# blyssprivacy/sdk

Measured on AMD Instinct MI355X. Metric: PIR queries/sec (full answer path) on 2^20 items x 256 B, higher is better.
Workload: dtype u64; 1 GPU; spiral-rs process_query, c2 = {"db_item_size": 256, "instances": 1, "n": 2, "nu_1": 9, "nu_2": 11, "p": 256, "q2_bits": 20, "t_conv": 4, "t_exp_left": 8, "t_exp_right": 56, "t_gsw": 8}, encoded DB 64.0 GiB (56.0 GiB resident per GPU), unsharded, one query per step

## Files before the change

### sdk_amd/csrc/fold.hip

```cpp
#include <type_traits>

#include "device_common.hpp"
#include "wave_ntt.hpp"
#include "bodies.hpp"

namespace spiral {

__device__ __forceinline__ bool fold_zero_shortcut(const u64* ct0, const u64* ct1, u64* out, int tau) {
  int nz0 = 0, nz1 = 0;
#pragma unroll
  for (int k = 0; k < 16; k++) {
    nz0 |= ct0[tau + 256 * k] != 0;
    nz1 |= ct1[tau + 256 * k] != 0;
  }
  const int any0 = __syncthreads_or(nz0), any1 = __syncthreads_or(nz1);
  if (any0 && any1) return false;
  const u64* src = any0 ? ct0 : ct1;
#pragma unroll
  for (int k = 0; k < 16; k++) out[tau + 256 * k] = src[tau + 256 * k];
  return true;
}

__global__ __launch_bounds__(256, 2) void k_fold_fused(DevTables T, FoldDesc d) {
  __shared__ u32 lds0[LDS_WORDS];
  __shared__ u32 lds1[LDS_WORDS];
  const int tau = threadIdx.x;
  const int i = (int)blockIdx.x, plane = blockIdx.y;
  const int two_t = 2 * d.t, four_t = 4 * d.t;
  const int t_live = d.t_live > 0 && d.t_live < d.t ? d.t_live : d.t;
  const u64* ct0 = d.X + ((size_t)plane * d.cur + i) * 2 * N;
  const u64* ct1 = ct0 + (size_t)d.half * 2 * N;
  const u64 mask = (1ULL << d.bits) - 1ULL;
  u32* la = lds0;
  u32* lb = lds1;
  u64* out = d.Y + ((size_t)plane * d.half + i) * 2 * N;
  if (d.zero_shortcuts && fold_zero_shortcut(ct0, ct1, out, tau)) return;
#pragma unroll 1
// ... 406 lines not shown
      } else {
#pragma unroll
        for (int kk = 0; kk < 16; kk++) mine_out[64 * kk + lt] = rr[kk];
      }
      __syncthreads();
      {
        const u32* theirs = exch + (irow * 2 + (1 - imod)) * (N / 2);
        u64* orow = out + (size_t)irow * N + (size_t)khalf * 1024;
        const u32 q0 = T.c.mod[0].q, q1 = T.c.mod[1].q;
        auto compose = [&](auto mod1_wave) {
          constexpr bool M1 = decltype(mod1_wave)::value;
#pragma unroll
          for (int kk = 0; kk < 16; kk++) {
            const u32 other = theirs[64 * kk + lt];
            const u32 own = rr[M1 ? kk : 16 + kk];
            const u32 x = M1 ? other : own, y = M1 ? own : other;
            const u32 xm = x >= q1 ? x - q1 : x;
            const u32 dd = y >= xm ? y - xm : y + q1 - xm;
            const u32 qt = __umulhi(dd, T.c.q0_inv_q1_sh);
            u32 e = dd * T.c.q0_inv_q1 - qt * q1;
            e = e >= q1 ? e - q1 : e;
            const u64 val = (u64)x + (u64)q0 * (u64)e + cpre[kk];
            const u64 res = val >= T.c.Q ? val - T.c.Q : val;
            orow[64 * kk + lt] = res;
          }
        };
        if (wv < 2) compose(std::true_type{});
        else compose(std::false_type{});
      }
    }
  }
}

__global__ __launch_bounds__(256, 2) void k_expand_wave(DevTables T, ExpandWaveDesc d, GroupOff g) {
  extern __shared__ __attribute__((aligned(16))) u32 smem_fw[];
  u32* wbuf = smem_fw;
  u32* ltw = smem_fw + 4 * WBUF_WORDS;
  u64* raw0 = reinterpret_cast<u64*>(ltw + 2 * N);
  const int tau = threadIdx.x, lane = tau & 63;
  const int wv = __builtin_amdgcn_readfirstlane(tau >> 6);
  const int b = (int)blockIdx.x, c = (int)blockIdx.y, qi = (int)blockIdx.z;
  const ModConst m = T.c.mod[c];
  const u32* fw = T.tw + (size_t)c * 4 * N;
  const u64* src = group_rebase(d.raw, g.raw[qi]) + (size_t)d.pos[b] * 2 * N;
  const u32* A_w = group_rebase(d.A_w, g.pp[qi]);
  u32* vout = group_rebase(d.v, g.v[qi]);
  u32* mybuf = wbuf + wv * WBUF_WORDS;
  wtw_stage(ltw, wave_fwd_image(T.tw, c), tau);
#pragma unroll
  for (int k = 0; k < 8; k++) raw0[tau + 256 * k] = src[tau + 256 * k];
  __syncthreads();
  const u64 mask = (1ULL << d.bits) - 1ULL;
  u64 acc0[32], acc1[32];
#pragma unroll
  for (int k = 0; k < 32; k++) acc0[k] = acc1[k] = 0;
#pragma unroll 1
  for (int dg = wv; dg <= d.t; dg += 4) {
    int ln = lane;
    const u32* fwi = fw;
    asm volatile("" : "+v"(ln));
    asm volatile("" : "+s"(fwi));
    WaveScalarTw stw;
    wntt_scalar_tw(stw, fwi);
    u32 v[32];
    if (dg < d.t) {
      const int sh = dg * d.bits;
// ... 54 lines not shown
      w.y = add_mod(wv == 0 ? r0[4 * g4 + 1] : r1[4 * g4 + 1], a.y, m.q);
      w.z = add_mod(wv == 0 ? r0[4 * g4 + 2] : r1[4 * g4 + 2], a.z, m.q);
      w.w = add_mod(wv == 0 ? r0[4 * g4 + 3] : r1[4 * g4 + 3], a.w, m.q);
      reinterpret_cast<uint4*>(o)[g4] = w;
    }
  }
}
void launch_expand_wave(const DevTables& T, const ExpandWaveDesc& d, const GroupOff& g, int B, hipStream_t s) {
  if (d.cnt <= 0 || B <= 0) return;
  const size_t lds = (size_t)(4 * WBUF_WORDS + 2 * N) * 4 + (size_t)N * 8;
  hipLaunchKernelGGL(k_expand_wave, dim3(d.cnt, 2, B), dim3(256), lds, s, T, d, g);
  launched(PATH_EXPAND_FUSED | PATH_EXPAND_WAVE, "k_expand_wave");
}

__global__ __launch_bounds__(256) void k_mats_to_wave(MatsToWaveDesc d) { mats_to_wave_body(d, blockIdx.x); }
void launch_mats_to_wave(u32* dst, const u32* src, size_t n_words, hipStream_t s, int half_polys) {
  if (n_words == 0) return;
  const MatsToWaveDesc d{dst, src, n_words, half_polys};
  hipLaunchKernelGGL(k_mats_to_wave, dim3((unsigned)((n_words + 255) / 256)), dim3(256), 0, s, d);
  launched(0, "k_mats_to_wave");
}

__global__ __launch_bounds__(256) void k_mats_to_wave_group(MatsToWaveDesc d, GroupOff g) {
  const int qi = blockIdx.y;
  d.dst = group_rebase(d.dst, g.raw[qi]);
  d.src = group_rebase(d.src, g.v[qi]);
  mats_to_wave_body(d, blockIdx.x);
}
void launch_mats_to_wave_group(u32* dst, const u32* src, size_t n_words, int half_polys, const GroupOff& g, int B, hipStream_t s) {
  if (n_words == 0 || B <= 0) return;
  const MatsToWaveDesc d{dst, src, n_words, half_polys};
  hipLaunchKernelGGL(k_mats_to_wave_group, dim3((unsigned)((n_words + 255) / 256), B), dim3(256), 0, s, d, g);
  launched(PATH_EXPAND_GROUP, "k_mats_to_wave_group");
}

void launch_fold_fused(const DevTables& T, const FoldDesc& d, hipStream_t s) {
  if (d.half <= 0 || d.planes <= 0) return;
  const int variant = (int)tunable("fold_variant", FOLD_VARIANT_DEFAULT);
  const dim3 grid(d.half, d.planes), block(256);
  if (variant == 5 && d.mats_w && d.bits <= 28) {
    const int es = d.bits <= 8 ? 1 : d.bits <= 16 ? 2 : 4;
    const int t_live = d.t_live > 0 && d.t_live < d.t ? d.t_live : d.t;
    const size_t lds = FOLD_WAVE_FIXED_LDS + (size_t)2 * t_live * (N * es + 256);
    if (lds <= 80 * 1024) {
      if (es == 1)
        hipLaunchKernelGGL(k_fold_wave<1>, grid, block, lds, s, T, d, d.mats_w);
      else if (es == 2)
        hipLaunchKernelGGL(k_fold_wave<2>, grid, block, lds, s, T, d, d.mats_w);
      else
        hipLaunchKernelGGL(k_fold_wave<4>, grid, block, lds, s, T, d, d.mats_w);
      launched(PATH_FOLD_FUSED | PATH_FOLD_WAVE, "k_fold_wave");
      return;
    }
  }
  if (variant != 0 && (d.t % 2) == 0)
    hipLaunchKernelGGL(k_fold_fused2, grid, block, 0, s, T, d);
  else
    hipLaunchKernelGGL(k_fold_fused, grid, block, 0, s, T, d);
  launched(PATH_FOLD_FUSED, "k_fold_fused");
}

}
```

### sdk_amd/csrc/kernels.hpp

```cpp
#pragma once
#include <hip/hip_runtime.h>

#include <vector>

#include "params.hpp"

namespace spiral {

constexpr int N = (int)POLY_LEN;

struct DevTables {
  const u32* tw;
  DevConsts c;
};
__host__ __device__ inline const u32* inv_tables(const u32* tw, int c) { return tw + (size_t)8 * N + (size_t)c * 2 * N; }
__host__ __device__ inline const u32* wave_fwd_image(const u32* tw, int c) { return tw + (size_t)12 * N + (size_t)c * 2 * N; }
__host__ __device__ inline int wtw_phys(int idx) {
  if (idx >= 1024) {
    const int L = (idx - 1024) >> 4, r = (idx - 1024) & 15;
    return 1024 + 16 * L + 4 * (((r >> 2) + (L >> 2)) & 3) + (r & 3);
  }
  if (idx >= 512) {
    const int L = (idx - 512) >> 3, r = (idx - 512) & 7;
    return 512 + 8 * L + 4 * (((r >> 2) + (L >> 3)) & 1) + (r & 3);
// ... 128 lines not shown
                               hipStream_t s);
void launch_reorient_group(u64* out, const u32* v, int first, int step, int dim0, const GroupOff& g, int B, hipStream_t s);
void launch_copy_polys_group(u32* dst, const int* dst_idx, int dst_row_stride, const u32* src, const int* src_idx, int src_row_stride,
                             int R, int batch, const GroupOff& g, int B, hipStream_t s);
void launch_folding_neg_group(const DevTables& T, u32* mats, const u32* gadget_ntt, int nu2, int two_t, const GroupOff& g, int B,
                              hipStream_t s);
void launch_mats_to_wave_group(u32* dst, const u32* src, size_t n_words, int half_polys, const GroupOff& g, int B, hipStream_t s);
struct ExpandWaveDesc {
  const u64* raw;
  const int* pos;
  const int* out_idx;
  const u32* A_w;
  const u32* const_w;
  u32* v;
  int cnt, t, bits;
};
void launch_expand_wave(const DevTables& T, const ExpandWaveDesc& d, const GroupOff& g, int B, hipStream_t s);
constexpr long EXPAND_WAVE_MIN_DIGITS_DEFAULT = 16;
constexpr long EXPAND_GROUP_ROUND_MIN_DEFAULT = 4096;

struct FoldDesc {
  const u64* X;
  u64* Y;
  const u32* mats;
  int cur, half, planes;
  int t, bits;
  int t_live;
  int zero_shortcuts;
  const u32* mats_w;
};
void launch_mats_to_wave(u32* dst, const u32* src, size_t n_words, hipStream_t s, int half_polys = 0);
constexpr long FOLD_VARIANT_DEFAULT = 5;
void launch_fold_fused(const DevTables& T, const FoldDesc& d, hipStream_t s);

void launch_add_poly_into(const DevTables& T, u32* dst, const int* idx, const u32* src, int batch, hipStream_t s);
void launch_scalar_mul(const DevTables& T, u32* base, long dst_off, long src_off, const u32* scalar, int n_polys,
                       hipStream_t s);
void launch_add_polys_idx(const DevTables& T, u32* dst, const int* di, const u32* a, const int* ai, const u32* b,
                          const int* bi, int count, hipStream_t s);
void launch_interleave_query(u64* qv, const u32* row0_ntt, const u64* wire, int dim0, hipStream_t s);
void launch_copy_polys(u32* dst, const int* dst_idx, int dst_row_stride, const u32* src, const int* src_idx,
                       int src_row_stride, int R, int batch, hipStream_t s);
void launch_folding_neg(const DevTables& T, u32* mats, const u32* gadget_ntt, int nu2, int two_t, hipStream_t s);
void launch_add(const DevTables& T, u32* out, const u32* a, const u32* b, int n_polys, hipStream_t s);
void launch_invert_raw(const DevTables& T, u64* out, const u64* a, long n_words, hipStream_t s);
void launch_automorph(const DevTables& T, u64* out, const u64* a, int n_polys, int t, hipStream_t s);
void launch_gadget_raw(u64* out, const u64* inp, int rows_in, int cols, int rows_out, int rdim, int bits,
                       hipStream_t s);
void launch_u64_to_u32(u32* out, const u64* in, long n, hipStream_t s);
void launch_u32_to_u64(u64* out, const u32* in, long n, hipStream_t s);

void launch_cu_probe(u32* out, int blocks, hipStream_t s);

struct EncodeDesc {
  const u64* packed;
  unsigned long long* out;
  int instances, n;
  u64 Q, q1, q2;
  int q1_bits, q2_bits;
};
void launch_encode(const EncodeDesc& d, hipStream_t s);

void launch_reorient(u64* out, const u32* v, int first, int step, int dim0, hipStream_t s);

struct CopyPolysDesc {
  u32* dst;
// ... 154 lines not shown
```

### sdk_amd/csrc/pipeline.hpp

```cpp
#pragma once
#include <vector>

#include "server.hpp"

namespace spiral {

struct Workspace {
  const Params* P;
  DeviceState* D;
  int device = -1;
  hipStream_t stream = nullptr;
  hipStream_t stream2 = nullptr;
  std::vector<hipEvent_t> ev_plane;
  hipEvent_t ev_fold = nullptr;
  hipEvent_t ev_round0 = nullptr, ev_right = nullptr;
  bool right_pending = false;
  bool long_sweep_follows = false;
  hipEvent_t ev_sw[2] = {nullptr, nullptr};
  bool have_sweep_span = false;
  bool pipelined = false;
  hipEvent_t ev[5] = {nullptr, nullptr, nullptr, nullptr, nullptr};
  DevBuf<u64> q_raw;
  DevBuf<u32> v;
  DevBuf<u64> exp_raw;
// ... 30 lines not shown
  ~Workspace();
  Workspace(const Workspace&) = delete;
  Workspace& operator=(const Workspace&) = delete;
  void ensure_expand();
  void ensure_sweep();
  void ensure_finish();
  size_t plane_group() const;
};

void run_coefficient_expansion(Workspace& W, const sp_pp& pp, size_t g_rounds, const DeviceState::PrunedPlan* plan = nullptr,
                               int tree = 0, size_t r_begin = 0);
void join_right(Workspace& W);
void run_regev_to_gsw(Workspace& W, const sp_pp& pp, const u32* v_src, const int* src_ct, const int* src_poly);
void run_folding_neg(Workspace& W);
void run_mats_to_wave(Workspace& W, size_t levels, bool c_only = false);
void run_fold_operands(Workspace& W);
void run_begin_direct(Workspace& W, const uint8_t* query);
void run_begin_group(Workspace* const* Ws, const sp_pp* const* pps, const uint8_t* const* queries, const size_t* query_lens, int B);
void run_begin(Workspace& W, const sp_pp& pp, const uint8_t* query, size_t query_len, int j0 = 0, int nj = 0,
               const DeviceState::PrunedPlan* plan = nullptr);
void run_sweep_sparse(Workspace& W, const sp_db& db, const int* col_ptr, const int* col_rows, const int* col_slots);
void run_sweep_sparse_group(Workspace* const* Ws, int B, const sp_db& db, const int* col_ptr, const int* col_rows, const int* col_slots,
                            hipStream_t s);
std::unique_ptr<DeviceState::PrunedPlan> build_pruned_plan_rows(const Params& P, const std::vector<char>& rows);
void run_sweep(Workspace& W, const sp_db& db);
void run_sweep_pipelined(Workspace& W, const sp_db& db);
bool sweep_is_pipelined(const Params& p, const sp_db& db);
void launch_plane_sweep(Workspace& W, const sp_db& db, size_t plane);
bool fused_fold_supported(const Params& p);
struct FoldOpts {
  long fused_min_pairs;
  bool delta_tail;
  bool inputs_below_q;
};
u64* run_fold(Workspace& W, const FoldOpts& o, u64* X, u64* Y, int np, int num_cts, int top, int d_begin = 0, int d_end = -1);
void run_fold_local(Workspace& W, const u32* reduced_chunk, int G);
void run_fold_local_plane(Workspace& W, const u32* reduced_plane_chunk, int G, int plane);
void run_fold_local_join(Workspace& W);
void run_finish_gathered(Workspace& W, const sp_pp& pp, const u64* gathered, int G);
void run_fold_all(Workspace& W, bool premod);
void run_pack(Workspace& W, const sp_pp& pp);
void run_finish(Workspace& W, const sp_pp& pp, bool premod);
size_t encode_response(const Params& p, const u64* packed, uint8_t* out);
void run_encode_device(Workspace& W);

}
```

### sdk_amd/csrc/server.cpp

```cpp
#include "server.hpp"

#include <algorithm>
#include <atomic>
#include <cstdlib>
#include <cstring>
#include <functional>

#include "pipeline.hpp"

namespace spiral {

void hip_check(hipError_t e, const char* what, const char* file, int line) {
  if (e != hipSuccess) {
    (void)hipGetLastError();
    throw HipError(std::string(what) + " failed at " + file + ":" + std::to_string(line) + ": " + hipGetErrorString(e));
  }
}

static std::mutex g_tun_mu;
static std::vector<std::pair<std::string, long>> g_tun;
static std::atomic<unsigned> g_tun_epoch{1};
static std::atomic<long> g_fresh_allocs{0};
void tunables_new_call() { g_tun_epoch.fetch_add(1, std::memory_order_relaxed); }
void set_tunable(const char* name, long v) {
// ... 1113 lines not shown
void join_right(Workspace& W) {
  if (W.right_pending) HIP_CHECK(hipStreamWaitEvent(W.stream, W.ev_right, 0));
}

void run_sweep(Workspace& W, const sp_db& db) {
  const Params& p = *W.P;
  W.ensure_sweep();
  SweepDesc d{db.words.p, W.qv.p, W.sweep_out.p, (int)p.planes(), db.np_local, (int)p.dim0(), db.j0, db.nj, db.packed, W.out_G};
  d.nt_store = (int)tunable("sweep_nt_store", 1);
  launch_sweep(W.D->T, d, W.stream);
}

void run_sweep_sparse(Workspace& W, const sp_db& db, const int* col_ptr, const int* col_rows, const int* col_slots) {
  const Params& p = *W.P;
  W.ensure_sweep();
  launch_sweep_sparse(W.D->T, col_ptr, col_rows, col_slots, db.polys.p, (int)p.planes(), W.v.p, 0,
                      p.db_dim_2 > 0 ? 2 : 1, W.sweep_out.p, (int)p.num_per(), W.stream);
}

void run_sweep_sparse_group(Workspace* const* Ws, int B, const sp_db& db, const int* col_ptr, const int* col_rows, const int* col_slots,
                            hipStream_t s) {
  const Params& p = *Ws[0]->P;
  SparseGroup g{};
  for (int b = 0; b < B; b++) {
    Ws[b]->ensure_sweep();
    g.v[b] = Ws[b]->v.p;
    g.out[b] = Ws[b]->sweep_out.p;
  }
  launch_sweep_sparse_batch(Ws[0]->D->T, col_ptr, col_rows, col_slots, db.polys.p, (int)p.planes(), g, B, 0, p.db_dim_2 > 0 ? 2 : 1,
                            (int)p.num_per(), s);
}

static FoldOpts query_fold_opts(const Workspace& W, bool below_q) {
  return FoldOpts{std::min(W.fused_min_pairs, tunable("fused_min_pairs_cap", 1L << 62)), true, below_q};
}

static void fold_planes(Workspace& W, size_t pg0, int np, bool premod) {
  const Params& p = *W.P;
  DeviceState& D = *W.D;
  hipStream_t s = W.stream;
  if (p.num_per() % 4 == 0 && !tunable("from_sweep1", 0)) {
    launch_from_sweep4(D.T, W.sweep_out.p + pg0 * 4 * POLY_LEN * p.num_per(), (int)p.num_per(), np, premod ? 1 : 0,
                       W.foldX.p, s);
  } else {
    InvDesc inv{};
    inv.src = W.sweep_out.p + pg0 * 4 * POLY_LEN * p.num_per();
    inv.sweep_np = (int)p.num_per();
    inv.dst = W.foldX.p;
    inv.n_polys = np * (int)p.num_per() * 2;
    inv.premod = premod ? 1 : 0;
    launch_ntt_inv(D.T, inv, s);
  }
  u64* res = run_fold(W, query_fold_opts(W, true), W.foldX.p, W.foldY.p, np, (int)p.num_per(), -1);
  HIP_CHECK(hipMemcpyAsync(W.final_cts.p + pg0 * 2 * POLY_LEN, res, (size_t)np * 2 * POLY_LEN * sizeof(u64), hipMemcpyDeviceToDevice, s));
}

static int tail_defer_levels(const Params& p, long stop) {
  if (stop <= 0 || !fused_fold_supported(p) || p.planes() < 2) return 0;
  int lv = 0;
  size_t cur = p.num_per();
  while (cur > (size_t)stop && cur / 2 >= 1 && (cur & 1) == 0) { cur >>= 1; lv++; }
  return cur == (size_t)stop && lv > 0 && stop >= 2 ? lv : 0;
}
static void fold_plane_head(Workspace& W, size_t pl, int levels) {
  const Params& p = *W.P;
  launch_from_sweep4(W.D->T, W.sweep_out.p + pl * 4 * POLY_LEN * p.num_per(), (int)p.num_per(), 1, 0, W.foldX.p, W.stream);
  u64* res = run_fold(W, query_fold_opts(W, true), W.foldX.p, W.foldY.p, 1, (int)p.num_per(), -1, 0, levels);
  const size_t cts = p.num_per() >> levels;
  HIP_CHECK(hipMemcpyAsync(W.fold_tail.p + pl * cts * 2 * POLY_LEN, res, cts * 2 * POLY_LEN * sizeof(u64), hipMemcpyDeviceToDevice, W.stream));
}
static void fold_tails(Workspace& W, int levels) {
  const Params& p = *W.P;
  const size_t cts = p.num_per() >> levels;
  u64* other = W.fold_tail.p + p.planes() * cts * 2 * POLY_LEN;
  u64* res = run_fold(W, query_fold_opts(W, true), W.fold_tail.p, other, (int)p.planes(), (int)p.num_per(), -1, levels, -1);
  HIP_CHECK(hipMemcpyAsync(W.final_cts.p, res, p.planes() * 2 * POLY_LEN * sizeof(u64), hipMemcpyDeviceToDevice, W.stream));
}

bool sweep_is_pipelined(const Params& p, const sp_db& db) {
  const bool enabled = tunable("pipeline", 1) != 0;
  return enabled && db.packed && db.num_shards == 1 && db.col_G == 1 && p.planes() > 1 && p.num_per() >= 1024;
}

void launch_plane_sweep(Workspace& W, const sp_db& db, size_t pl) {
  const Params& p = *W.P;
  const size_t np_ = (size_t)db.np_local;
  const size_t plane_db_words = db_bytes(1, db.np_local, db.nj, db.packed) / 8;
  SweepDesc d{db.words.p + pl * plane_db_words, W.qv.p, W.sweep_out.p + pl * 4 * POLY_LEN * np_, 1, db.np_local,
              (int)p.dim0(), db.j0, db.nj, db.packed, W.out_G};
  d.nt_store = (int)tunable("sweep_nt_store", 1);
  const int wgs = (int)tunable("pipe_wgs", 4);
  if (db.packed && wgs > 0)
    launch_sweep_persist(W.D->T, d, wgs, W.stream);
  else
    launch_sweep(W.D->T, d, W.stream);
}

void run_sweep_pipelined(Workspace& W, const sp_db& db) {
  const Params& p = *W.P;
  W.ensure_sweep();
  W.ensure_finish();
  const size_t planes = p.planes();
  HIP_CHECK(hipEventRecord(W.ev_sw[0], W.stream));
  const int defer_levels = tail_defer_levels(p, tunable("pipe_tail_defer", 256));
  if (defer_levels > 0) {
    W.fold_tail.ensure(2 * planes * (p.num_per() >> defer_levels) * 2 * POLY_LEN);
    note_path(PATH_FOLD_TAIL_BATCHED);
  }
  for (size_t pl = 0; pl < planes; pl++) {
    launch_plane_sweep(W, db, pl);
    HIP_CHECK(hipEventRecord(W.ev_plane[pl], W.stream));
    HIP_CHECK(hipStreamWaitEvent(W.stream2, W.ev_plane[pl], 0));
    if (defer_levels > 0) {
      on_stream(W, W.stream2, [&] {
        fold_plane_head(W, pl, defer_levels);
        if (pl + 1 == planes) fold_tails(W, defer_levels);
      });
      continue;
    }
    on_stream(W, W.stream2, [&] { fold_planes(W, pl, 1, false); });
  }
  HIP_CHECK(hipEventRecord(W.ev_sw[1], W.stream));
  HIP_CHECK(hipEventRecord(W.ev_fold, W.stream2));
  W.have_sweep_span = true;
  W.pipelined = true;
  note_path(PATH_PIPELINED);
}

bool fused_fold_supported(const Params& p) { return 4 * p.t_gsw <= 128 && p.bits_per(p.t_gsw) <= 28; }

u64* run_fold(Workspace& W, const FoldOpts& o, u64* X, u64* Y, int np, int num_cts, int top, int d_begin, int d_end) {
  const Params& p = *W.P;
  DeviceState& D = *W.D;
  hipStream_t s = W.stream;
  const int two_t = (int)(2 * p.t_gsw);
  join_right(W);
  int further = 0;
  while (((int)1 << further) < num_cts) further++;
  const int top_idx = top < 0 ? further - 1 : top;
  if (d_end < 0) d_end = further;
  int cur = num_cts >> d_begin;
  for (int d = d_begin; d < d_end; d++) {
    const int half = cur / 2;
    if (W.zero_shortcuts && !fused_fold_supported(p))
      throw ArgError("sparse buckets need gadget parameters the fused fold supports (3 <= t_gsw <= 32)");
    if (W.zero_shortcuts || ((long)np * half >= o.fused_min_pairs && fused_fold_supported(p))) {
      FoldDesc fd{};
      fd.zero_shortcuts = W.zero_shortcuts ? 1 : 0;
      fd.mats_w = W.mats_w_ready ? W.fold_mats_w.p + (size_t)(top_idx - d) * 2 * 2 * two_t * 2 * POLY_LEN : nullptr;
      fd.X = X;
      fd.Y = Y;
      fd.mats = W.fold_mats.p + (size_t)(top_idx - d) * 2 * 2 * two_t * 2 * POLY_LEN;
      fd.cur = cur;
      fd.half = half;
      fd.planes = np;
      fd.t = (int)p.t_gsw;
      fd.bits = (int)p.bits_per(p.t_gsw);
      fd.t_live = o.inputs_below_q && tunable("fold_skip_dead_digits", 1)
                      ? (int)std::min<size_t>(p.t_gsw, (p.modulus_log2 + fd.bits - 1) / fd.bits) : fd.t;
      launch_fold_fused(D.T, fd, s);
      std::swap(X, Y);
      cur = half;
      continue;
    }
    if (o.delta_tail) {
      FwdDesc f{};
      f.src = X;
      f.dst = W.fold_dig.p;
      f.n_out = np * half * two_t;
      f.rdim = 2;
      f.cols = 1;
      f.t = (int)p.t_gsw;
      f.bits = (int)p.bits_per(p.t_gsw);
      f.src_batch_stride = 2;
      f.src_row0 = 0;
      f.src_cols = 1;
      f.delta_off = (long)half * 2;
      f.delta_inner = half;
      f.delta_outer_stride = cur;
// ... 37 lines not shown
    f.t = (int)p.t_gsw;
    f.bits = (int)p.bits_per(p.t_gsw);
    f.src_batch_stride = 2;
    f.src_row0 = 0;
    f.src_cols = 1;
    launch_ntt_fwd(D.T, f, s);
    MacDesc m{};
    m.A = W.fold_mats.p + (size_t)(top_idx - d) * 2 * 2 * two_t * 2 * POLY_LEN;
    m.B = W.fold_dig.p;
    m.out = W.fold_ntt.p;
    m.R = 2;
    m.K = 2 * two_t;
    m.batch_inner = half;
    m.batch_outer = np;
    m.B_inner_stride = two_t;
    m.B_outer_stride = (long)cur * two_t;
    m.split_k = two_t;
    m.split_off = (long)half * two_t;
    m.out_batch_stride = 2;
    m.out_row_stride = 1;
    launch_mac(D.T, m, s);
    InvDesc inv{};
    inv.src = W.fold_ntt.p;
    inv.poly_stride = 2 * POLY_LEN;
    inv.crt_stride = POLY_LEN;
    inv.z_stride = 1;
    inv.dst = Y;
    inv.n_polys = np * half * 2;
    launch_ntt_inv(D.T, inv, s);
    note_path(PATH_FOLD_TAIL_LITERAL);
    std::swap(X, Y);
    cur = half;
  }
  return X;
}

static void run_pack_v1(Workspace& W, const sp_pp& pp) {
  const Params& p = *W.P;
  DeviceState& D = *W.D;
  hipStream_t s = W.stream;
  const int* L = D.lists.p;
  const int tc = (int)p.t_conv;
  note_path(PATH_PACK_V1);
  const int nb = (int)p.planes();
  const int ne = (int)p.instances * 2;
  const size_t PW = 2 * POLY_LEN;
  W.pack_v1_P.ensure((size_t)nb * 3 * PW);
  W.pack_v1_P2.ensure((size_t)ne * 3 * PW);
  W.pack_v1_raw.ensure((size_t)ne * POLY_LEN);
  const u32* w_key = pp.all.p + (pp.off_packing + 0 * 3 * tc) * PW;
  const u32* w_shift = pp.all.p + (pp.off_packing + 1 * 3 * tc) * PW;
  FwdDesc f{};
  f.src = W.final_cts.p;
  f.src_idx = L + D.pack_src_ct;
  f.dst = W.pack_dig.p;
  f.n_out = nb * tc;
  f.rdim = 1; f.cols = 1; f.t = tc; f.bits = (int)p.bits_per(tc);
  f.src_batch_stride = 2; f.src_row0 = 0; f.src_cols = 1;
  launch_ntt_fwd(D.T, f, s);
  MacDesc m{};
  m.A = w_key; m.B = W.pack_dig.p; m.out = W.pack_v1_P.p;
  m.R = 3; m.K = tc; m.batch_inner = nb; m.batch_outer = 1; m.B_inner_stride = tc; m.split_k = tc;
  m.out_batch_stride = 3; m.out_row_stride = 1;
  launch_mac(D.T, m, s);
  FwdDesc f2 = f;
  f2.dst = W.pack_ct2.p; f2.n_out = nb; f2.t = 1; f2.bits = 64; f2.src_row0 = 1;
// ... 110 lines not shown
    val &= (nbits >= 64) ? ~0ULL : (((u64)1 << nbits) - 1);
    size_t wi = bit >> 6, off = bit & 63;
    words[wi] |= val << off;
    if (off + nbits > 64) words[wi + 1] |= val >> (64 - off);
    bit += nbits;
  };
  const size_t mat = (p.n + 1) * p.n * POLY_LEN;
  for (size_t inst = 0; inst < p.instances; inst++) {
    const u64* m = packed + inst * mat;
    for (size_t i = 0; i < p.n * POLY_LEN; i++) put(rescale_coeff(m[i], p.modulus, q2), q2_bits);
    const u64* rest = m + p.n * POLY_LEN;
    for (size_t i = 0; i < p.n * p.n * POLY_LEN; i++) put(rescale_coeff(rest[i], p.modulus, q1), q1_bits);
  }
  memcpy(out, words.data(), total);
  return total;
}

static void fold_local_planes(Workspace& W, const u32* chunk, int G, size_t pg0, int np) {
  const Params& p = *W.P;
  DeviceState& D = *W.D;
  hipStream_t s = W.stream;
  const int npl = (int)p.num_per() / G;
  if (npl % 4 == 0) {
    launch_from_sweep4(D.T, chunk, npl, np, 1, W.foldX.p, s);
  } else {
    InvDesc inv{};
    inv.src = chunk;
    inv.sweep_np = npl;
    inv.dst = W.foldX.p;
    inv.n_polys = np * npl * 2;
    inv.premod = 1;
    launch_ntt_inv(D.T, inv, s);
  }
  u64* res = run_fold(W, query_fold_opts(W, true), W.foldX.p, W.foldY.p, np, npl, (int)p.db_dim_2 - 1);
  HIP_CHECK(hipMemcpyAsync(W.final_cts.p + pg0 * 2 * POLY_LEN, res, (size_t)np * 2 * POLY_LEN * sizeof(u64), hipMemcpyDeviceToDevice, s));
}

void run_fold_local(Workspace& W, const u32* reduced_chunk, int G) {
  const Params& p = *W.P;
  W.ensure_finish();
  const int npl = (int)p.num_per() / G;
  const size_t pg = W.plane_group();
  for (size_t pg0 = 0; pg0 < p.planes(); pg0 += pg)
    fold_local_planes(W, reduced_chunk + pg0 * 4 * POLY_LEN * npl, G, pg0, (int)std::min(pg, p.planes() - pg0));
}

void run_fold_local_plane(Workspace& W, const u32* reduced_plane_chunk, int G, int plane) {
  W.ensure_finish();
  std::swap(W.stream, W.stream2);
  try {
    fold_local_planes(W, reduced_plane_chunk, G, (size_t)plane, 1);
  } catch (...) {
    std::swap(W.stream, W.stream2);
    throw;
  }
  std::swap(W.stream, W.stream2);
}

void run_fold_local_join(Workspace& W) {
  HIP_CHECK(hipEventRecord(W.ev_fold, W.stream2));
  HIP_CHECK(hipStreamWaitEvent(W.stream, W.ev_fold, 0));
}

void run_finish_gathered(Workspace& W, const sp_pp& pp, const u64* gathered, int G) {
  const Params& p = *W.P;
  hipStream_t s = W.stream;
  W.ensure_finish();
  const size_t ctw = 2 * POLY_LEN;
  const int planes = (int)p.planes();
  W.foldX.ensure((size_t)planes * G * ctw);
  W.foldY.ensure((size_t)planes * std::max(G / 2, 1) * ctw);
  HIP_CHECK(hipMemcpy2DAsync(W.foldX.p, (size_t)G * ctw * 8, gathered, ctw * 8, ctw * 8, (size_t)planes, hipMemcpyDeviceToDevice, s));
  for (int g = 1; g < G; g++)
    HIP_CHECK(hipMemcpy2DAsync(W.foldX.p + (size_t)g * ctw, (size_t)G * ctw * 8, gathered + (size_t)g * planes * ctw, ctw * 8,
                               ctw * 8, (size_t)planes, hipMemcpyDeviceToDevice, s));
  int lg = 0;
  while ((1 << lg) < G) lg++;
  u64* res = run_fold(W, query_fold_opts(W, false), W.foldX.p, W.foldY.p, planes, G, lg - 1);
  HIP_CHECK(hipMemcpyAsync(W.final_cts.p, res, (size_t)planes * ctw * sizeof(u64), hipMemcpyDeviceToDevice, s));
  HIP_CHECK(hipEventRecord(W.ev[3], s));
  run_pack(W, pp);
  run_encode_device(W);
  HIP_CHECK(hipEventRecord(W.ev[4], s));
}

void run_encode_device(Workspace& W) {
  const Params& p = *W.P;
  hipStream_t s = W.stream;
  HIP_CHECK(hipMemsetAsync(W.enc_out.p, 0, W.enc_out.bytes(), s));
  EncodeDesc e{};
  e.packed = W.pack_raw.p;
  e.out = reinterpret_cast<unsigned long long*>(W.enc_out.p);
  e.instances = (int)p.instances;
  e.n = (int)p.n;
  e.Q = p.modulus;
  e.q1 = 4 * p.pt_modulus;
  e.q2 = p.q2();
  int q1_bits = 0;
  while (((u64)1 << q1_bits) < e.q1) q1_bits++;
  e.q1_bits = q1_bits;
  e.q2_bits = (int)p.q2_bits;
  launch_encode(e, s);
  HIP_CHECK(hipMemcpyAsync(W.h_response, W.enc_out.p, p.response_bytes(), hipMemcpyDeviceToHost, s));
}

void run_finish(Workspace& W, const sp_pp& pp, bool premod) {
  const Params& p = *W.P;
  W.ensure_finish();
  if (W.pipelined) {
    HIP_CHECK(hipStreamWaitEvent(W.stream, W.ev_fold, 0));
    W.pipelined = false;
  } else {
// ... 11 lines not shown
```

Before: 92.66 queries/s.

## Add wide 512-thread tail fold kernel keeping residues between small fold levels

Adds a fold kernel for the small late levels of the fold (few ciphertext pairs). It uses 8 waves per block and one block per CRT modulus, spreading the gadget digit products across waves and combining them with an LDS tree reduction. Between consecutive wide levels the data stays in split residue form, and a separate compose kernel runs only at the end, writing straight into the final destination so the trailing device copy is skipped. This aims to fix poor GPU occupancy in the tail levels. In exchange it uses a large LDS footprint, several extra block barriers and extra launch paths.

After: 92.99 queries/s, median of 6. About the same (+0.4%).

```diff
diff --git a/sdk_amd/csrc/fold.hip b/sdk_amd/csrc/fold.hip
--- a/sdk_amd/csrc/fold.hip
+++ b/sdk_amd/csrc/fold.hip
@@ -3,6 +3,7 @@
 #include "device_common.hpp"
 #include "wave_ntt.hpp"
 #include "bodies.hpp"
+#include "server.hpp"
 
 namespace spiral {
 
@@ -475,6 +476,10 @@
   }
 }
 
+}
+#include "fold_wide.hpp"
+namespace spiral {
+
 __global__ __launch_bounds__(256, 2) void k_expand_wave(DevTables T, ExpandWaveDesc d, GroupOff g) {
   extern __shared__ __attribute__((aligned(16))) u32 smem_fw[];
   u32* wbuf = smem_fw;
@@ -595,6 +600,32 @@
   const MatsToWaveDesc d{dst, src, n_words, half_polys};
   hipLaunchKernelGGL(k_mats_to_wave_group, dim3((unsigned)((n_words + 255) / 256), B), dim3(256), 0, s, d, g);
   launched(PATH_EXPAND_GROUP, "k_mats_to_wave_group");
+}
+
+bool fold_tail_wide_takes(int bits, int t_live) { return tail_wide_takes(bits, t_live); }
+void launch_fold_tail_wide(const DevTables& T, const FoldDesc& d, bool in_res, hipStream_t s) {
+  if (d.half <= 0 || d.planes <= 0) return;
+  const int t_live = d.t_live > 0 && d.t_live < d.t ? d.t_live : d.t;
+  if (!d.mats_w || !tail_wide_takes(d.bits, t_live)) throw ArgError("launch_fold_tail_wide: gadget width not taken");
+  const size_t lds = tail_wide_lds(d.bits, t_live);
+  const dim3 grid(d.half, d.planes, 2), block(TAIL_WIDE_THREADS);
+  const int es = tail_wide_es(d.bits);
+#define SP_TAIL_WIDE(ES_)                                                                                               \
+  {                                                                                                                     \
+            \
+    if (lds > 65536)                                                                                                    \
+      HIP_CHECK(hipFuncSetAttribute(reinterpret_cast<const void*>(&k_tail_wide<ES_>),                                   \
+                                    hipFuncAttributeMaxDynamicSharedMemorySize, (int)lds));                             \
+    hipLaunchKernelGGL(k_tail_wide<ES_>, grid, block, lds, s, T, d, d.mats_w, in_res ? 1 : 0);                          \
+  }
+  if (es == 1) SP_TAIL_WIDE(1) else if (es == 2) SP_TAIL_WIDE(2) else SP_TAIL_WIDE(4)
+#undef SP_TAIL_WIDE
+  launched(PATH_FOLD_TAIL | PATH_FOLD_TAIL_PERSIST, "k_tail_wide");
+}
+void launch_fold_tail_compose(const DevTables& T, const u64* src, u64* dst, int cts, hipStream_t s) {
+  if (cts <= 0) return;
+  hipLaunchKernelGGL(k_tail_compose, dim3(cts), dim3(256), 0, s, T, reinterpret_cast<const u32*>(src), dst);
+  launched(0, "k_tail_compose");
 }
 
 void launch_fold_fused(const DevTables& T, const FoldDesc& d, hipStream_t s) {
diff --git a/sdk_amd/csrc/fold_wide.hpp b/sdk_amd/csrc/fold_wide.hpp
--- /dev/null
+++ b/sdk_amd/csrc/fold_wide.hpp
@@ -0,0 +1,235 @@
+#pragma once
+#include "device_common.hpp"
+#include "wave_ntt.hpp"
+
+namespace spiral {
+
+constexpr int TAIL_WIDE_WAVES = 8;
+constexpr int TAIL_WIDE_THREADS = 64 * TAIL_WIDE_WAVES;
+constexpr int TAIL_WIDE_FIXED_LDS = (TAIL_WIDE_WAVES * WBUF_WORDS + 2 * N) * 4;
+constexpr int TAIL_WIDE_SCRATCH_LDS = (TAIL_WIDE_WAVES / 2) * 2 * N * 4;
+constexpr int TAIL_WIDE_MAX_LDS = 160 * 1024;
+constexpr int TAIL_WIDE_MAX_PRODUCTS = 21;
+
+__host__ __device__ inline int tail_wide_es(int bits) { return bits <= 8 ? 1 : bits <= 16 ? 2 : 4; }
+inline size_t tail_wide_lds(int bits, int t_live) {
+  const size_t lds = TAIL_WIDE_FIXED_LDS + (size_t)2 * t_live * (N * tail_wide_es(bits) + 256);
+  return lds < (size_t)TAIL_WIDE_SCRATCH_LDS ? (size_t)TAIL_WIDE_SCRATCH_LDS : lds;
+}
+inline bool tail_wide_takes(int bits, int t_live) {
+  return bits >= 1 && bits < 28 && t_live >= 1 && tail_wide_lds(bits, t_live) <= (size_t)TAIL_WIDE_MAX_LDS &&
+         (2 * t_live + TAIL_WIDE_WAVES - 1) / TAIL_WIDE_WAVES <= TAIL_WIDE_MAX_PRODUCTS;
+}
+
+__device__ __forceinline__ u64 tail_compose(u32 x, u32 y, const DevConsts& c) {
+  const u32 q1 = c.mod[1].q;
+  const u32 xm = x >= q1 ? x - q1 : x;
+  const u32 dd = y >= xm ? y - xm : y + q1 - xm;
+  const u32 qt = __umulhi(dd, c.q0_inv_q1_sh);
+  u32 e = dd * c.q0_inv_q1 - qt * q1;
+  e = e >= q1 ? e - q1 : e;
+  return (u64)x + (u64)c.mod[0].q * (u64)e;
+}
+
+template <int ES>
+__global__ __launch_bounds__(TAIL_WIDE_THREADS) void k_tail_wide(DevTables T, FoldDesc d, const u32* __restrict__ mats_w, int in_res) {
+  extern __shared__ __attribute__((aligned(16))) u32 smem_fw[];
+  u32* wbuf = smem_fw;
+  u32* ltw = smem_fw + TAIL_WIDE_WAVES * WBUF_WORDS;
+  const int t_live = d.t_live > 0 && d.t_live < d.t ? d.t_live : d.t;
+  unsigned char* dig = reinterpret_cast<unsigned char*>(ltw + 2 * N);
+  unsigned char* sgn = dig + (size_t)2 * t_live * (N * ES);
+  constexpr int E = 16 / ES;
+  const int tau = threadIdx.x, lane = tau & 63;
+  const int wv = __builtin_amdgcn_readfirstlane(tau >> 6);
+  const int i = (int)blockIdx.x, plane = blockIdx.y, c = (int)blockIdx.z;
+  const int two_t = 2 * d.t, four_t = 4 * d.t;
+  const u64* ct0 = d.X + ((size_t)plane * d.cur + i) * 2 * N;
+  const u64* ct1 = ct0 + (size_t)d.half * 2 * N;
+  u32* out = reinterpret_cast<u32*>(d.Y + ((size_t)plane * d.half + i) * 2 * N);
+  const ModConst m = T.c.mod[c];
+  const u32* fw = T.tw + (size_t)c * 4 * N;
+  u32* mybuf = wbuf + wv * WBUF_WORDS;
+  {
+    const u32x4w_t* img = reinterpret_cast<const u32x4w_t*>(wave_fwd_image(T.tw, c));
+#pragma unroll
+    for (int k = 0; k < 2; k++) reinterpret_cast<u32x4w_t*>(ltw)[tau + TAIL_WIDE_THREADS * k] = img[tau + TAIL_WIDE_THREADS * k];
+  }
+  {
+    const int j = wv >> 2, kg = wv & 3;
+    const u64 mask = (1ULL << d.bits) - 1ULL;
+    u64 x0[8], x1[8];
+    if (in_res) {
+      const u32* r0 = reinterpret_cast<const u32*>(ct0) + (size_t)j * 2 * N;
+      const u32* r1 = reinterpret_cast<const u32*>(ct1) + (size_t)j * 2 * N;
+      u32 a0[8], b0[8], a1[8], b1[8];
+#pragma unroll
+      for (int e = 0; e < 8; e++) {
+        const int n = 64 * (8 * kg + e) + lane;
+        a0[e] = r0[n]; b0[e] = r0[N + n];
+        a1[e] = r1[n]; b1[e] = r1[N + n];
+      }
+#pragma unroll
+      for (int e = 0; e < 8; e++) {
+        x0[e] = tail_compose(a0[e], b0[e], T.c);
+        x1[e] = tail_compose(a1[e], b1[e], T.c);
+      }
+    } else {
+#pragma unroll
+      for (int e = 0; e < 8; e++) {
+        const size_t n = (size_t)j * N + 64 * (8 * kg + e) + lane;
+        x0[e] = ct0[n];
+        x1[e] = ct1[n];
+      }
+    }
+#pragma unroll 1
+    for (int kd = 0; kd < t_live; kd++) {
+      const int sh = (kd * d.bits) & 63;
+      const u64 dmask = kd * d.bits >= 64 ? 0ULL : mask;
+      u32 df[8];
+#pragma unroll
+      for (int e = 0; e < 8; e++) df[e] = (u32)((x1[e] >> sh) & dmask) - (u32)((x0[e] >> sh) & dmask);
+      unsigned char* base = dig + (size_t)(j * t_live + kd) * (N * ES);
+      u32 sb = 0;
+#pragma unroll
+      for (int e = 0; e < 8; e++) sb |= (df[e] >> 31) << e;
+      sgn[(j * t_live + kd) * 256 + lane * 4 + kg] = (unsigned char)sb;
+      if (ES == 1) {
+        u32x2w_t o;
+        o.x = (df[0] & 0xff) | ((df[1] & 0xff) << 8) | ((df[2] & 0xff) << 16) | (df[3] << 24);
+        o.y = (df[4] & 0xff) | ((df[5] & 0xff) << 8) | ((df[6] & 0xff) << 16) | (df[7] << 24);
+        *reinterpret_cast<u32x2w_t*>(base + (kg >> 1) * 1024 + lane * 16 + 8 * (kg & 1)) = o;
+      } else if (ES == 2) {
+        u32x4w_t o;
+        o.x = (df[0] & 0xffff) | (df[1] << 16); o.y = (df[2] & 0xffff) | (df[3] << 16);
+        o.z = (df[4] & 0xffff) | (df[5] << 16); o.w = (df[6] & 0xffff) | (df[7] << 16);
+        *reinterpret_cast<u32x4w_t*>(base + kg * 1024 + lane * 16) = o;
+      } else {
+        u32x4w_t o;
+        o.x = df[0]; o.y = df[1]; o.z = df[2]; o.w = df[3];
+        *reinterpret_cast<u32x4w_t*>(base + (2 * kg) * 1024 + lane * 16) = o;
+        o.x = df[4]; o.y = df[5]; o.z = df[6]; o.w = df[7];
+        *reinterpret_cast<u32x4w_t*>(base + (2 * kg + 1) * 1024 + lane * 16) = o;
+      }
+    }
+  }
+  __syncthreads();
+  u64 acc0[32], acc1[32];
+#pragma unroll
+  for (int k = 0; k < 32; k++) acc0[k] = acc1[k] = 0;
+#pragma unroll 1
+  for (int dg = wv; dg < 2 * t_live; dg += TAIL_WIDE_WAVES) {
+    const int j = dg / t_live, kd = dg - j * t_live;
+    int ln = lane;
+    const u32* fwi = fw;
+    asm volatile("" : "+v"(ln));
+    asm volatile("" : "+s"(fwi));
+    const unsigned char* src = dig + (size_t)dg * (N * ES) + ln * 16;
+    u32x4w_t dv[2 * ES];
+#pragma unroll
+    for (int h = 0; h < 2 * ES; h++) dv[h] = *reinterpret_cast<const u32x4w_t*>(src + h * 1024);
+    const int sg = *reinterpret_cast<const int*>(sgn + dg * 256 + ln * 4);
+    WaveScalarTw stw;
+    wntt_scalar_tw(stw, fwi);
+    SP_SB();
+    u32 v[32];
+#pragma unroll
+    for (int h = 0; h < 2 * ES; h++) {
+      const u32 wd[4] = {dv[h].x, dv[h].y, dv[h].z, dv[h].w};
+#pragma unroll
+      for (int e = 0; e < E; e++) {
+        const int sm = __builtin_amdgcn_sbfe(sg, h * E + e, 1);
+        const int sd = ES == 4 ? (int)wd[e] : (int)(__builtin_amdgcn_ubfe(wd[(e * ES) >> 2], ((e * ES) & 3) * 8, 8 * ES) | ((u32)sm << (8 * ES)));
+        v[h * E + e] = (u32)(sd + (sm & (int)m.q));
+      }
+    }
+    const int kk = two_t + j + 2 * kd;
+    FoldMac hk{acc0, acc1, reinterpret_cast<const u32x4w_t*>(mats_w + ((size_t)kk * 2 + c) * N) + ln,
+               reinterpret_cast<const u32x4w_t*>(mats_w + ((size_t)(four_t + kk) * 2 + c) * N) + ln};
+    wntt_fwd<false>(v, ln, mybuf, fwi, stw, ltw, m.q, m.two_q, hk);
+  }
+  int lt = lane;
+  asm volatile("" : "+v"(lt));
+  u32 r0[32], r1[32];
+#pragma unroll
+  for (int k = 0; k < 32; k++) {
+    r0[k] = reduce64(acc0[k], m);
+    r1[k] = reduce64(acc1[k], m);
+  }
+  u64 cpre[32];
+  if (wv < 2) {
+    if (in_res) {
+      const u32* crow = reinterpret_cast<const u32*>(ct0) + (size_t)wv * 2 * N + (size_t)c * N;
+#pragma unroll
+      for (int k = 0; k < 32; k++) cpre[k] = crow[64 * k + lt];
+    } else {
+      const u64* crow = ct0 + (size_t)wv * N;
+#pragma unroll
+      for (int k = 0; k < 32; k++) cpre[k] = crow[64 * k + lt];
+    }
+  }
+  u32x4w_t* sc = reinterpret_cast<u32x4w_t*>(smem_fw);
+#define SP_PUT(R, REGION)                                                                              \
+_Pragma("unroll") for (int g = 0; g < 8; g++) {                                                      \
+  u32x4w_t t4;                                                                                       \
+  t4.x = R[4 * g]; t4.y = R[4 * g + 1]; t4.z = R[4 * g + 2]; t4.w = R[4 * g + 3];                    \
+  sc[(REGION) * 512 + g * 64 + lt] = t4;                                                             \
+}
+#define SP_ADD(R, REGION)                                                                              \
+_Pragma("unroll") for (int g = 0; g < 8; g++) {                                                      \
+  const u32x4w_t t4 = sc[(REGION) * 512 + g * 64 + lt];                                              \
+  R[4 * g] = add_mod(R[4 * g], t4.x, m.q); R[4 * g + 1] = add_mod(R[4 * g + 1], t4.y, m.q);          \
+  R[4 * g + 2] = add_mod(R[4 * g + 2], t4.z, m.q); R[4 * g + 3] = add_mod(R[4 * g + 3], t4.w, m.q);  \
+}
+  __syncthreads();
+  if (wv >= 4) { SP_PUT(r0, 2 * (wv - 4)) SP_PUT(r1, 2 * (wv - 4) + 1) }
+  __syncthreads();
+  if (wv < 4) { SP_ADD(r0, 2 * wv) SP_ADD(r1, 2 * wv + 1) }
+  __syncthreads();
+  if (wv < 4) {
+    if (wv & 1) { SP_PUT(r0, wv) } else { SP_PUT(r1, wv) }
+  }
+  __syncthreads();
+  if (wv < 4) {
+    if (wv & 1) { SP_ADD(r1, wv - 1) } else { SP_ADD(r0, wv + 1) }
+  }
+  __syncthreads();
+  if (wv == 2) { SP_PUT(r0, 0) }
+  if (wv == 3) { SP_PUT(r1, 1) }
+  __syncthreads();
+  if (wv == 0) { SP_ADD(r0, 0) }
+  if (wv == 1) { SP_ADD(r1, 1) }
+  __syncthreads();
+#undef SP_PUT
+#undef SP_ADD
+  if (wv < 2) {
+    u32 rr[32];
+#pragma unroll
+    for (int k = 0; k < 32; k++) rr[k] = wv == 0 ? r0[k] : r1[k];
+    u32 cres[32];
+#pragma unroll
+    for (int k = 0; k < 32; k++) cres[k] = reduce64(cpre[k], m);
+    wntt_inv(rr, lt, mybuf, inv_tables(T.tw, c), m.q, m.two_q);
+    u32* orow = out + (size_t)wv * 2 * N + (size_t)c * N;
+#pragma unroll
+    for (int k = 0; k < 32; k++) orow[64 * k + lt] = add_mod(rr[k], cres[k], m.q);
+  }
+}
+
+__global__ __launch_bounds__(256) void k_tail_compose(DevTables T, const u32* src, u64* dst) {
+  const int tau = threadIdx.x;
+  const u32* s = src + (size_t)blockIdx.x * 4 * N;
+  u64* o = dst + (size_t)blockIdx.x * 2 * N;
+  u64 val[16];
+#pragma unroll
+  for (int r = 0; r < 2; r++)
+#pragma unroll
+    for (int k = 0; k < 8; k++) val[8 * r + k] = tail_compose(s[(size_t)r * 2 * N + tau + 256 * k], s[(size_t)r * 2 * N + N + tau + 256 * k], T.c);
+  __syncthreads();
+#pragma unroll
+  for (int r = 0; r < 2; r++)
+#pragma unroll
+    for (int k = 0; k < 8; k++) o[(size_t)r * N + tau + 256 * k] = val[8 * r + k];
+}
+
+}
diff --git a/sdk_amd/csrc/kernels.hpp b/sdk_amd/csrc/kernels.hpp
--- a/sdk_amd/csrc/kernels.hpp
+++ b/sdk_amd/csrc/kernels.hpp
@@ -184,6 +184,10 @@
 void launch_mats_to_wave(u32* dst, const u32* src, size_t n_words, hipStream_t s, int half_polys = 0);
 constexpr long FOLD_VARIANT_DEFAULT = 5;
 void launch_fold_fused(const DevTables& T, const FoldDesc& d, hipStream_t s);
+bool fold_tail_wide_takes(int bits, int t_live);
+void launch_fold_tail_wide(const DevTables& T, const FoldDesc& d, bool in_res, hipStream_t s);
+void launch_fold_tail_compose(const DevTables& T, const u64* src, u64* dst, int cts, hipStream_t s);
+constexpr long FOLD_TAIL_WIDE_MAX_DEFAULT = 128;
 
 void launch_add_poly_into(const DevTables& T, u32* dst, const int* idx, const u32* src, int batch, hipStream_t s);
 void launch_scalar_mul(const DevTables& T, u32* base, long dst_off, long src_off, const u32* scalar, int n_polys,
diff --git a/sdk_amd/csrc/pipeline.hpp b/sdk_amd/csrc/pipeline.hpp
--- a/sdk_amd/csrc/pipeline.hpp
+++ b/sdk_amd/csrc/pipeline.hpp
@@ -86,8 +86,10 @@
   long fused_min_pairs;
   bool delta_tail;
   bool inputs_below_q;
+  long wide_fused_max = 0;
 };
-u64* run_fold(Workspace& W, const FoldOpts& o, u64* X, u64* Y, int np, int num_cts, int top, int d_begin = 0, int d_end = -1);
+u64* run_fold(Workspace& W, const FoldOpts& o, u64* X, u64* Y, int np, int num_cts, int top, int d_begin = 0, int d_end = -1,
+              u64* final_dst = nullptr);
 void run_fold_local(Workspace& W, const u32* reduced_chunk, int G);
 void run_fold_local_plane(Workspace& W, const u32* reduced_plane_chunk, int G, int plane);
 void run_fold_local_join(Workspace& W);
diff --git a/sdk_amd/csrc/server.cpp b/sdk_amd/csrc/server.cpp
--- a/sdk_amd/csrc/server.cpp
+++ b/sdk_amd/csrc/server.cpp
@@ -1169,7 +1169,7 @@
 }
 
 static FoldOpts query_fold_opts(const Workspace& W, bool below_q) {
-  return FoldOpts{std::min(W.fused_min_pairs, tunable("fused_min_pairs_cap", 1L << 62)), true, below_q};
+  return FoldOpts{std::min(W.fused_min_pairs, tunable("fused_min_pairs_cap", 1L << 62)), true, below_q, 0};
 }
 
 static void fold_planes(Workspace& W, size_t pg0, int np, bool premod) {
@@ -1188,8 +1188,9 @@
     inv.premod = premod ? 1 : 0;
     launch_ntt_inv(D.T, inv, s);
   }
-  u64* res = run_fold(W, query_fold_opts(W, true), W.foldX.p, W.foldY.p, np, (int)p.num_per(), -1);
-  HIP_CHECK(hipMemcpyAsync(W.final_cts.p + pg0 * 2 * POLY_LEN, res, (size_t)np * 2 * POLY_LEN * sizeof(u64), hipMemcpyDeviceToDevice, s));
+  u64* dst = W.final_cts.p + pg0 * 2 * POLY_LEN;
+  u64* res = run_fold(W, query_fold_opts(W, true), W.foldX.p, W.foldY.p, np, (int)p.num_per(), -1, 0, -1, dst);
+  if (res != dst) HIP_CHECK(hipMemcpyAsync(dst, res, (size_t)np * 2 * POLY_LEN * sizeof(u64), hipMemcpyDeviceToDevice, s));
 }
 
 static int tail_defer_levels(const Params& p, long stop) {
@@ -1210,8 +1211,10 @@
   const Params& p = *W.P;
   const size_t cts = p.num_per() >> levels;
   u64* other = W.fold_tail.p + p.planes() * cts * 2 * POLY_LEN;
-  u64* res = run_fold(W, query_fold_opts(W, true), W.fold_tail.p, other, (int)p.planes(), (int)p.num_per(), -1, levels, -1);
-  HIP_CHECK(hipMemcpyAsync(W.final_cts.p, res, p.planes() * 2 * POLY_LEN * sizeof(u64), hipMemcpyDeviceToDevice, W.stream));
+  FoldOpts o = query_fold_opts(W, true);
+  o.wide_fused_max = tunable("fold_tails_wide_fused_max", 0);
+  u64* res = run_fold(W, o, W.fold_tail.p, other, (int)p.planes(), (int)p.num_per(), -1, levels, -1, W.final_cts.p);
+  if (res != W.final_cts.p) HIP_CHECK(hipMemcpyAsync(W.final_cts.p, res, p.planes() * 2 * POLY_LEN * sizeof(u64), hipMemcpyDeviceToDevice, W.stream));
 }
 
 bool sweep_is_pipelined(const Params& p, const sp_db& db) {
@@ -1266,12 +1269,19 @@
 
 bool fused_fold_supported(const Params& p) { return 4 * p.t_gsw <= 128 && p.bits_per(p.t_gsw) <= 28; }
 
-u64* run_fold(Workspace& W, const FoldOpts& o, u64* X, u64* Y, int np, int num_cts, int top, int d_begin, int d_end) {
+u64* run_fold(Workspace& W, const FoldOpts& o, u64* X, u64* Y, int np, int num_cts, int top, int d_begin, int d_end, u64* final_dst) {
   const Params& p = *W.P;
   DeviceState& D = *W.D;
   hipStream_t s = W.stream;
   const int two_t = (int)(2 * p.t_gsw);
   join_right(W);
+  const int fold_bits = (int)p.bits_per(p.t_gsw);
+  const int fold_t_live = o.inputs_below_q && tunable("fold_skip_dead_digits", 1)
+                              ? (int)std::min<size_t>(p.t_gsw, (p.modulus_log2 + fold_bits - 1) / fold_bits) : (int)p.t_gsw;
+  const bool wide_ok = tunable("fold_tail_wide", 1) != 0 && o.delta_tail && !W.zero_shortcuts && W.mats_w_ready &&
+                       fused_fold_supported(p) && fold_tail_wide_takes(fold_bits, fold_t_live);
+  const long wide_max = tunable("fold_tail_wide_max", FOLD_TAIL_WIDE_MAX_DEFAULT);
+  bool resid = false;
   int further = 0;
   while (((int)1 << further) < num_cts) further++;
   const int top_idx = top < 0 ? further - 1 : top;
@@ -1281,7 +1291,31 @@
     const int half = cur / 2;
     if (W.zero_shortcuts && !fused_fold_supported(p))
       throw ArgError("sparse buckets need gadget parameters the fused fold supports (3 <= t_gsw <= 32)");
-    if (W.zero_shortcuts || ((long)np * half >= o.fused_min_pairs && fused_fold_supported(p))) {
+    const long steps = (long)np * half;
+    const bool fused_level = W.zero_shortcuts || (steps >= o.fused_min_pairs && fused_fold_supported(p));
+    if (wide_ok && steps <= (fused_level ? o.wide_fused_max : wide_max)) {
+      FoldDesc fd{};
+      fd.mats_w = W.fold_mats_w.p + (size_t)(top_idx - d) * 2 * 2 * two_t * 2 * POLY_LEN;
+      fd.X = X;
+      fd.Y = Y;
+      fd.mats = W.fold_mats.p + (size_t)(top_idx - d) * 2 * 2 * two_t * 2 * POLY_LEN;
+      fd.cur = cur;
+      fd.half = half;
+      fd.planes = np;
+      fd.t = (int)p.t_gsw;
+      fd.bits = fold_bits;
+      fd.t_live = fold_t_live;
+      launch_fold_tail_wide(D.T, fd, resid, s);
+      resid = true;
+      std::swap(X, Y);
+      cur = half;
+      continue;
+    }
+    if (resid) {
+      launch_fold_tail_compose(D.T, X, X, np * cur, s);
+      resid = false;
+    }
+    if (fused_level) {
       FoldDesc fd{};
       fd.zero_shortcuts = W.zero_shortcuts ? 1 : 0;
       fd.mats_w = W.mats_w_ready ? W.fold_mats_w.p + (size_t)(top_idx - d) * 2 * 2 * two_t * 2 * POLY_LEN : nullptr;
@@ -1385,6 +1419,11 @@
     std::swap(X, Y);
     cur = half;
   }
+  if (resid) {
+    u64* dst = final_dst ? final_dst : X;
+    launch_fold_tail_compose(D.T, X, dst, np * cur, s);
+    return dst;
+  }
   return X;
 }
 
@@ -1561,8 +1600,9 @@
     inv.premod = 1;
     launch_ntt_inv(D.T, inv, s);
   }
-  u64* res = run_fold(W, query_fold_opts(W, true), W.foldX.p, W.foldY.p, np, npl, (int)p.db_dim_2 - 1);
-  HIP_CHECK(hipMemcpyAsync(W.final_cts.p + pg0 * 2 * POLY_LEN, res, (size_t)np * 2 * POLY_LEN * sizeof(u64), hipMemcpyDeviceToDevice, s));
+  u64* dst = W.final_cts.p + pg0 * 2 * POLY_LEN;
+  u64* res = run_fold(W, query_fold_opts(W, true), W.foldX.p, W.foldY.p, np, npl, (int)p.db_dim_2 - 1, 0, -1, dst);
+  if (res != dst) HIP_CHECK(hipMemcpyAsync(dst, res, (size_t)np * 2 * POLY_LEN * sizeof(u64), hipMemcpyDeviceToDevice, s));
 }
 
 void run_fold_local(Workspace& W, const u32* reduced_chunk, int G) {
@@ -1605,8 +1645,8 @@
                                ctw * 8, (size_t)planes, hipMemcpyDeviceToDevice, s));
   int lg = 0;
   while ((1 << lg) < G) lg++;
-  u64* res = run_fold(W, query_fold_opts(W, false), W.foldX.p, W.foldY.p, planes, G, lg - 1);
-  HIP_CHECK(hipMemcpyAsync(W.final_cts.p, res, (size_t)planes * ctw * sizeof(u64), hipMemcpyDeviceToDevice, s));
+  u64* res = run_fold(W, query_fold_opts(W, false), W.foldX.p, W.foldY.p, planes, G, lg - 1, 0, -1, W.final_cts.p);
+  if (res != W.final_cts.p) HIP_CHECK(hipMemcpyAsync(W.final_cts.p, res, (size_t)planes * ctw * sizeof(u64), hipMemcpyDeviceToDevice, s));
   HIP_CHECK(hipEventRecord(W.ev[3], s));
   run_pack(W, pp);
   run_encode_device(W);
```
